# marcomistretta/incremental_multimodal_medical_learning_II

Hardware: AMD Instinct MI355X
Metric: contrastive train-step images/sec at global batch 1024; 1/2/4/8-GPU scaling (higher is better)
Workload: dtype bf16x3

## Files before the change

### incremental_multimodal_medical_learning_ii_amd/csrc/conv_wgrad.hip

```cpp
#include "conv_common.h"

using namespace cxrk;

namespace {
__global__ __launch_bounds__(256) void wgrad_reduce_bn_kernel(const float* __restrict__ slabs, int nslab, long slab_stride,
                                                              int taps, int C, int Cpad, const float* __restrict__ w,
                                                              const float* __restrict__ scale, float* __restrict__ dw,
                                                              float* __restrict__ dotpart, int accumulate, int sg_log2) {
  __shared__ float sh[16];
  __shared__ float4 red[256];
  const int ko = blockIdx.x;
  const int n = taps * Cpad;
  const float sc = scale ? scale[ko] : 1.f;
  const int SG = 1 << sg_log2, QPB = 256 >> sg_log2;
  const int ql = threadIdx.x & (QPB - 1), grp = threadIdx.x >> (8 - sg_log2);
  const int i4 = (blockIdx.y * QPB + ql) * 4;
  float4 s = make_float4(0.f, 0.f, 0.f, 0.f);
  if (i4 < n) {
    const float* src = slabs + (long)ko * n + i4;
    int z = grp;
    for (; z + 3 * SG < nslab; z += 4 * SG) {
      const float4 t0 = *reinterpret_cast<const float4*>(src + (long)z * slab_stride);
      const float4 t1 = *reinterpret_cast<const float4*>(src + (long)(z + SG) * slab_stride);
      const float4 t2 = *reinterpret_cast<const float4*>(src + (long)(z + 2 * SG) * slab_stride);
      const float4 t3 = *reinterpret_cast<const float4*>(src + (long)(z + 3 * SG) * slab_stride);
      s.x += (t0.x + t1.x) + (t2.x + t3.x); s.y += (t0.y + t1.y) + (t2.y + t3.y);
      s.z += (t0.z + t1.z) + (t2.z + t3.z); s.w += (t0.w + t1.w) + (t2.w + t3.w);
    }
    for (; z < nslab; z += SG) {
      const float4 t = *reinterpret_cast<const float4*>(src + (long)z * slab_stride);
      s.x += t.x; s.y += t.y; s.z += t.z; s.w += t.w;
    }
  }
  if (SG > 1) {
    red[threadIdx.x] = s;
    __syncthreads();
    if (grp == 0) {
      for (int g2 = 1; g2 < SG; ++g2) { const float4 t = red[g2 * QPB + ql]; s.x += t.x; s.y += t.y; s.z += t.z; s.w += t.w; }
    }
  }
  float dot = 0.f;
  if (i4 < n && grp == 0) {
    const int tap = i4 / Cpad, c = i4 - tap * Cpad;
    const float sv[4] = {s.x, s.y, s.z, s.w};
#pragma unroll
    for (int q = 0; q < 4; ++q) {
      if (c + q < C) {
        const long o = ((long)ko * taps + tap) * C + c + q;
        if (dotpart) dot += w[o] * sv[q];
        dw[o] = accumulate ? dw[o] + sc * sv[q] : sc * sv[q];
      }
    }
  }
  if (dotpart) {
    dot = block_sum(dot, sh);
    if (threadIdx.x == 0) dotpart[(long)ko * gridDim.y + blockIdx.y] = dot;
  }
}
__global__ void bn_param_grad_kernel(const float* __restrict__ dotpart, int nparts, const float* __restrict__ rstd,
                                     const float* __restrict__ rmean, const float* __restrict__ sumdy, int Ko,
                                     float* __restrict__ dgamma, float* __restrict__ dbeta, int accumulate) {
  const int ko = blockIdx.x * blockDim.x + threadIdx.x;
  if (ko >= Ko) return;
  float dot = 0.f;
  for (int p = 0; p < nparts; ++p) dot += dotpart[(long)ko * nparts + p];
  const float g = rstd[ko] * (dot - rmean[ko] * sumdy[ko]);
  dgamma[ko] = accumulate ? dgamma[ko] + g : g;
  dbeta[ko] = accumulate ? dbeta[ko] + sumdy[ko] : sumdy[ko];
}

}

static int wgrad_splitk(int Ko, int Ncols, long Kred, bool planes) { return wgrad_splitk_policy(Ko, Ncols, (int)Kred, planes); }
static int wgrad_dot_parts(int Nc) { return ceil_div(Nc, 64); }

extern "C" size_t cxrk_conv_wgrad_ws_bytes(int N, int H, int W, int C, int Ko, int R, int S, int stride, int pad) {
  const ConvGeom g = make_geom(N, H, W, C, Ko, R, S, stride, pad);
  int sk = wgrad_splitk(Ko, R * S * C, (long)N * g.Ho * g.Wo, false);
  const int sk2 = wgrad_splitk(Ko, R * S * C, (long)N * g.Ho * g.Wo, true);
  if (sk2 > sk) sk = sk2;
  return ((size_t)sk * (size_t)Ko * (size_t)(R * S * C) + (size_t)Ko * wgrad_dot_parts(R * S * C)) * sizeof(float);
}

template <class FMT>
static int conv_bwd_params_impl(const typename FMT::T* x, long xplane, const typename FMT::T* dy, long dyplane, const float* w,
                                const float* scale, const float* rstd, const float* rmean, const float* sumdy, float* dw,
                                float* dgamma, float* dbeta, int accumulate, int N, int H, int W, int C, int Cpad, int Ko, int R,
                                int S, int stride, int pad, float* ws, size_t ws_bytes, hipStream_t stream) {
  CXRK_CHECK_ARG(x && dy && dw && N > 0 && Cpad % FMT::EPL == 0 && Ko % FMT::EPL == 0 && aligned16(x) && aligned16(dy));
  CXRK_CHECK_ARG(!(dgamma && !(w && rstd && rmean && sumdy && dbeta)));
  const ConvGeom g = make_geom(N, H, W, Cpad, Ko, R, S, stride, pad);
  const long Kl = (long)N * g.Ho * g.Wo;
  CXRK_CHECK_ARG(Kl < (1L << 31));
  const int Kred = (int)Kl, Nc = R * S * Cpad;
  if ((long)H * W * Cpad * 4 * 3 >= (1L << 31)) return CXRK_ERR_UNSUPPORTED;
  int sk = wgrad_splitk(Ko, Nc, Kl, FMT::PLANES);
  const size_t slab_floats = (size_t)sk * Ko * Nc;
  CXRK_CHECK_WS(ws, ws_bytes, (slab_floats + (size_t)Ko * wgrad_dot_parts(Nc)) * sizeof(float));
  EpiParams ep{};
  ep.C = ws; ep.ldc = Nc; ep.alpha = 1.f; ep.slab_stride = (long)Ko * Nc;
  int rc;
  const bool exact = false;
  if (use_wide256(Ko, Nc, Kred, sk, FMT::PLANES)) {
    if constexpr (FMT::PLANES) {
      DmaDenseMC<256, 8>::P pa{dy, (long)Ko, Ko, Kred, dyplane}; DmaConvIm2colMC<256, 8>::P pb{x, g, Nc, Kred, xplane};
      rc = launch_gemm_pw<Pw256, DmaDenseMC<256, 8>, DmaConvIm2colMC<256, 8>>(pa, pb, ep, Ko, Nc, Kred, sk, stream);
    } else return CXRK_ERR_UNSUPPORTED;
  } else if (Ko <= 64) {
    if constexpr (FMT::PLANES) {
      DmaDenseMC<64, 4>::P pa{dy, (long)Ko, Ko, Kred, dyplane}; DmaConvIm2colMC<256, 4>::P pb{x, g, Nc, Kred, xplane};
      rc = launch_gemm_pw<Pw64x256, DmaDenseMC<64, 4>, DmaConvIm2colMC<256, 4>>(pa, pb, ep, Ko, Nc, Kred, sk, stream);
    } else {
      typename DenseMC<64, FMT>::P pa{dy, (long)Ko, Ko, Kred, dyplane}; typename ConvIm2colMC<256, FMT>::P pb{x, g, Nc, Kred, xplane};
      rc = launch_gemm<DenseMC<64, FMT>, ConvIm2colMC<256, FMT>, 1, 4>(pa, pb, ep, Ko, Nc, Kred, sk, stream, exact);
    }
  } else if constexpr (FMT::PLANES) {
    DmaDenseMC<128, 4>::P pa{dy, (long)Ko, Ko, Kred, dyplane}; DmaConvIm2colMC<128, 4>::P pb{x, g, Nc, Kred, xplane};
    rc = launch_gemm_pw<Pw128, DmaDenseMC<128, 4>, DmaConvIm2colMC<128, 4>>(pa, pb, ep, Ko, Nc, Kred, sk, stream);
  } else {
    typename DenseMC<128, FMT>::P pa{dy, (long)Ko, Ko, Kred, dyplane}; typename ConvIm2colMC<128, FMT>::P pb{x, g, Nc, Kred, xplane};
    rc = launch_gemm<DenseMC<128, FMT>, ConvIm2colMC<128, FMT>, 2, 2>(pa, pb, ep, Ko, Nc, Kred, sk, stream, exact);
  }
  if (rc < 0) return rc;
  const int sg_log2 = rc >= 64 ? 4 : (rc >= 8 ? 2 : 0);
  const int ny = ceil_div(Nc, 4 * (256 >> sg_log2));
  float* dotpart = dgamma ? ws + slab_floats : nullptr;
  hipLaunchKernelGGL(wgrad_reduce_bn_kernel, dim3(Ko, ny), dim3(256), 0, stream, ws, rc, (long)Ko * Nc, R * S, C, Cpad, w, scale, dw,
                     dotpart, accumulate, sg_log2);
  CXRK_LAUNCH_CHECK();
  if (dgamma) {
    hipLaunchKernelGGL(bn_param_grad_kernel, dim3(ceil_div(Ko, 256)), dim3(256), 0, stream, dotpart, ny, rstd, rmean, sumdy, Ko, dgamma,
                       dbeta, accumulate);
    CXRK_LAUNCH_CHECK();
  }
  return CXRK_OK;
}

extern "C" int cxrk_conv_bn_act_bwd_params(const float* x, const float* dy, const float* w, const float* scale,
                                           const float* rstd, const float* rmean, const float* sumdy, float* dw,
                                           float* dgamma, float* dbeta, int accumulate, int N, int H, int W, int C,
                                           int Cpad, int Ko, int R, int S, int stride, int pad, float* ws, size_t ws_bytes,
                                           hipStream_t stream) {
  return conv_bwd_params_impl<F32>(x, 0, dy, 0, w, scale, rstd, rmean, sumdy, dw, dgamma, dbeta, accumulate, N, H, W, C, Cpad, Ko, R, S,
                                   stride, pad, ws, ws_bytes, stream);
}
extern "C" int cxrk_conv_bn_act_bwd_params_pl(const void* x, long xplane, const void* dy, long dyplane, const float* w,
                                              const float* scale, const float* rstd, const float* rmean, const float* sumdy,
                                              float* dw, float* dgamma, float* dbeta, int accumulate, int N, int H, int W, int C,
                                              int Ko, int R, int S, int stride, int pad, float* ws, size_t ws_bytes,
                                              hipStream_t stream) {
  return conv_bwd_params_impl<PL>(static_cast<const unsigned short*>(x), xplane, static_cast<const unsigned short*>(dy), dyplane, w, scale,
                                  rstd, rmean, sumdy, dw, dgamma, dbeta, accumulate, N, H, W, C, C, Ko, R, S, stride, pad, ws, ws_bytes,
                                  stream);
}
```

### incremental_multimodal_medical_learning_ii_amd/kernels.py

```python
from __future__ import annotations

from typing import NamedTuple, Optional, Tuple

import torch

from . import _lib
from ._lib import check

ACT_NONE, ACT_RELU, ACT_GELU = 0, 1, 2
AUX_NONE, AUX_RELU_MASK, AUX_GELU_GRAD, AUX_MASK_BITS = 0, 1, 2, 3


def _stream() -> int:
    return torch.cuda.current_stream().cuda_stream


def _p(t: Optional[torch.Tensor]) -> Optional[int]:
    return None if t is None else t.data_ptr()


def _chk(t: torch.Tensor, name: str, dtype=torch.float32) -> torch.Tensor:
    if not isinstance(t, torch.Tensor) or not t.is_cuda:
        raise ValueError(f"{name}: expected a tensor on the GPU (the cxrk path has no CPU fallback), got "
                         f"{type(t).__name__} on {getattr(t, 'device', None)}")
    if t.dtype != dtype:
        raise ValueError(f"{name}: expected dtype {dtype}, got {t.dtype}")
    return t


def _chk_out(t, shape, name: str, dtype=torch.float32):
    if isinstance(t, Planes):
        if tuple(t.shape) != tuple(shape) or not t.is_contiguous():
            raise ValueError(f"{name}: expected contiguous Planes of shape {tuple(shape)}, got {tuple(t.shape)}")
        return t
    _chk(t, name, dtype)
    if tuple(t.shape) != tuple(shape) or not t.is_contiguous():
        raise ValueError(f"{name}: expected a contiguous tensor of shape {tuple(shape)}, got {tuple(t.shape)} strides {t.stride()}")
    return t


def _rowmajor2d(t: torch.Tensor, name: str) -> Tuple[torch.Tensor, int]:
    _chk(t, name)
    if t.dim() != 2:
        raise ValueError(f"{name}: expected 2-D, got shape {tuple(t.shape)}")
    if t.shape[1] != 1 and t.stride(1) != 1:
        t = t.contiguous()
    return t, (t.stride(0) if t.shape[0] > 1 else max(t.shape[1], t.stride(0)))


class Planes:
    __slots__ = ("t",)

    def __init__(self, t: torch.Tensor):
        if t.dtype != torch.bfloat16 or t.dim() < 2 or t.shape[0] != 2 or not t.is_cuda:
            raise ValueError(f"Planes: expected a bf16 GPU tensor [2, ...], got {t.dtype} {tuple(t.shape)} on {t.device}")
        self.t = t

    @staticmethod
    def empty(*shape, device) -> "Planes":
        return Planes(torch.empty((2,) + tuple(shape), dtype=torch.bfloat16, device=device))

    @staticmethod
    def zeros(*shape, device) -> "Planes":
        return Planes(torch.zeros((2,) + tuple(shape), dtype=torch.bfloat16, device=device))

    @property
    def shape(self):
        return self.t.shape[1:]

    @property
    def device(self):
        return self.t.device

    @property
    def plane(self) -> int:
        return self.t.stride(0)

    def ptr(self) -> int:
        return self.t.data_ptr()

    def numel(self) -> int:
        return self.t.numel() // 2

    def view(self, *shape) -> "Planes":
        return Planes(self.t.view((2,) + tuple(shape)))

    def rows(self, sl) -> "Planes":
        return Planes(self.t[:, sl])

    def is_contiguous(self) -> bool:
        return self.t[0].is_contiguous()

    def float(self) -> torch.Tensor:
        if self.is_contiguous() and self.numel() % 8 == 0:
            out = torch.empty(tuple(self.shape), dtype=torch.float32, device=self.t.device)
            check(_lib.load().cxrk_merge_planes(self.ptr(), self.plane, self.numel(), _p(out), _stream()), "cxrk_merge_planes")
            return out
        return self.t[0].float() + self.t[1].float()


def split_planes(x: torch.Tensor, out: Optional[Planes] = None) -> Planes:
    _chk(x, "split_planes.x")
    x = x.contiguous()
    if out is None:
        out = Planes.empty(*x.shape, device=x.device)
    check(_lib.load().cxrk_split_planes(_p(x), x.numel(), out.ptr(), out.plane, _stream()), "cxrk_split_planes")
    return out


def _pl2d(t: Planes, name: str):
    if not isinstance(t, Planes) or len(t.shape) != 2:
        raise ValueError(f"{name}: expected a 2-D Planes tensor")
    v = t.t
    if v.shape[2] != 1 and v.stride(2) != 1:
        raise ValueError(f"{name}: planes columns must be contiguous")
    return v.data_ptr(), (v.stride(1) if v.shape[1] > 1 else max(v.shape[2], v.stride(1))), v.stride(0)


class LaunchProfiler:

    PEAK_BF16X3, PEAK_F32, PEAK_HBM = 2500e12 / 3.0, 157.3e12, 8.0e12

    def __init__(self):
        self.on = False
        self.rows = []

    def start(self):
        self.on, self.rows = True, []

    def stop(self):
        self.on = False

    def bracket(self, key: str, flops: float, nbytes: float = 0.0, sub: int = 1):
        if not self.on:
            return None
        a, b = torch.cuda.Event(enable_timing=True), torch.cuda.Event(enable_timing=True)
        a.record()
        self.rows.append((key, flops, nbytes, a, b, sub))
        return b

    def summary(self):
        out = {}
        for key, flops, nbytes, a, b, sub in self.rows:
            d = out.setdefault(key, {"launches": 0, "flops": 0.0, "bytes": 0.0, "ms": 0.0, "floor_ms": 0.0})
            d["launches"] += sub
            d["flops"] += flops
            d["bytes"] += nbytes
            d["ms"] += a.elapsed_time(b)
            peak = self.PEAK_BF16X3 if (key.startswith("gemm_pw") or key.startswith("gemm_x3")) else self.PEAK_F32
            d["floor_ms"] += 1e3 * max(flops / peak, nbytes / self.PEAK_HBM)
        return out


profiler = LaunchProfiler()
# ... 359 lines not shown
    op, opl = _fmt(dz, "bn_train_dz.dz")
    check(lib.cxrk_bn_train_dz(dp, dpl, zp, zpl, _p(_vec(A, C, "A")), _p(_vec(B, C, "B")), _p(_vec(Cc, C, "Cc")), op, opl, rows, C, _stream()),
          "cxrk_bn_train_dz")
    return dz



def bn_fold(w, gamma, beta, rmean, rvar, eps, Ko, taps, C, Cpad, w_scaled, scale, shift, rstd):
    lib = _lib.load()
    for n, t in (("w", w), ("gamma", gamma), ("beta", beta), ("rmean", rmean), ("rvar", rvar)):
        _chk(t, "bn_fold." + n)
    check(lib.cxrk_bn_fold(_p(w), _p(gamma), _p(beta), _p(rmean), _p(rvar), float(eps), Ko, taps, C, Cpad,
                           _p(w_scaled), _p(scale), _p(shift), _p(rstd), _stream()), "cxrk_bn_fold")


def conv_fwd(x, w_scaled, shift, residual, y, N, H, W, C, Ko, R, S, stride, pad, relu):
    lib = _lib.load()
    ev = None
    if profiler.on:
        Ho, Wo = (H + 2 * pad - R) // stride + 1, (W + 2 * pad - S) // stride + 1
        fl = 2.0 * N * Ho * Wo * Ko * R * S * C
        ev = profiler.bracket(_label("ConvIm2colKC", "DenseKC", "4,1" if Ko <= 64 else "2,2", N * Ho * Wo, Ko, R * S * C, 1,
                                     1 if C % 32 == 0 else 3), fl,
                              4.0 * (N * H * W * C + Ko * R * S * C + N * Ho * Wo * Ko * (1 + (residual is not None))))
    rc = lib.cxrk_conv_bn_act_fwd(_p(_chk(x, "conv.x")), _p(w_scaled), _p(shift), _p(residual), _p(y), N, H, W, C, Ko,
                                  R, S, stride, pad, int(relu), _stream())
    if ev is not None:
        ev.record()
    check(rc, f"cxrk_conv_bn_act_fwd(N={N},H={H},W={W},C={C},Ko={Ko},R={R},s={stride})")
    return y


def _conv_out(H, W, R, S, stride, pad):
    return (H + 2 * pad - R) // stride + 1, (W + 2 * pad - S) // stride + 1


def _dgrad_label(N, H, W, Ko, R, S, stride):
    if stride == 1:
        return "ConvDgradKC", "ConvFilterMC", N * H * W, R * S * Ko, 1
    classes = 4 if R > 1 else 1
    return "ConvDgradS2KC", "ConvFilterS2MC", N * ((H + 1) // 2) * ((W + 1) // 2), Ko * max(1, (R * S) // 4), classes


def conv_bwd_data(dy, w_scaled, residual, relu_src, dx, N, H, W, C, Ko, R, S, stride, pad, sums=None):
    lib = _lib.load()
    ws = workspace(lib.cxrk_conv_bwd_data_colsum_ws_bytes(N, H, W, C, stride), dy.device) if sums is not None else None
    ev = None
    if profiler.on:
        Ho, Wo = _conv_out(H, W, R, S, stride, pad)
        fl = 2.0 * N * Ho * Wo * Ko * R * S * C
        la, lb, Ml, Kl, sub = _dgrad_label(N, H, W, Ko, R, S, stride)
        ev = profiler.bracket(_label(la, lb, "4,1" if C <= 64 else "2,2", Ml, C, Kl, 1, 2), fl,
                              4.0 * (N * Ho * Wo * Ko + Ko * R * S * C + N * H * W * C * (1 + (residual is not None) + (relu_src is not None))), sub)
    rc = lib.cxrk_conv_bn_act_bwd_data(_p(_chk(dy, "conv.dy")), _p(w_scaled), _p(residual), _p(relu_src), _p(dx), N, H,
                                       W, C, Ko, R, S, stride, pad, _p(sums), _p(ws), ws.numel() * 4 if ws is not None else 0, _stream())
    if ev is not None:
        ev.record()
    check(rc, f"cxrk_conv_bn_act_bwd_data(N={N},H={H},W={W},C={C},Ko={Ko},R={R},s={stride})")
    return dx


def conv_bwd_params(x, dy, w, scale, rstd, rmean, sumdy, dw, dgamma, dbeta, accumulate, N, H, W, C, Cpad, Ko, R, S, stride, pad):
    lib = _lib.load()
    wsb = lib.cxrk_conv_wgrad_ws_bytes(N, H, W, Cpad, Ko, R, S, stride, pad)
    ws = workspace(wsb, x.device)
    ev = None
    if profiler.on:
        Ho, Wo = _conv_out(H, W, R, S, stride, pad)
        fl = 2.0 * N * Ho * Wo * Ko * R * S * Cpad
        sk = lib.cxrk_gemm_wgrad_splitk(Ko, R * S * Cpad, N * Ho * Wo, 0)
        ev = profiler.bracket(_label("DenseMC", "ConvIm2colMC", "1,4" if Ko <= 64 else "2,2", Ko, R * S * Cpad, N * Ho * Wo, sk, 0,
                                     False), fl, 4.0 * (N * H * W * Cpad + N * Ho * Wo * Ko + Ko * R * S * Cpad))
    check(lib.cxrk_conv_bn_act_bwd_params(_p(_chk(x, "conv.x")), _p(_chk(dy, "conv.dy")), _p(w), _p(scale), _p(rstd),
                                          _p(rmean), _p(sumdy), _p(dw), _p(dgamma), _p(dbeta), int(accumulate), N, H, W,
                                          C, Cpad, Ko, R, S, stride, pad, _p(ws), ws.numel() * 4, _stream()),
          f"cxrk_conv_bn_act_bwd_params(N={N},H={H},W={W},C={C},Ko={Ko},R={R},s={stride})")
    if ev is not None:
        ev.record()



def bn_fold_pl(w, gamma, beta, rmean, rvar, eps, Ko, taps, C, Cpad, w_scaled: Planes, scale, shift, rstd):
    lib = _lib.load()
    for n, t in (("w", w), ("gamma", gamma), ("beta", beta), ("rmean", rmean), ("rvar", rvar)):
        _chk(t, "bn_fold." + n)
    check(lib.cxrk_bn_fold_pl(_p(w), _p(gamma), _p(beta), _p(rmean), _p(rvar), float(eps), Ko, taps, C, Cpad, w_scaled.ptr(),
                              w_scaled.plane, _p(scale), _p(shift), _p(rstd), _stream()), "cxrk_bn_fold_pl")


def conv_fwd_pl(x, w_scaled, shift, residual: Optional[Planes], y: Planes, maskout, N, H, W, C, Ko, R, S, stride, pad, relu):
    lib = _lib.load()
    in_planes = isinstance(x, Planes)
    if in_planes != isinstance(w_scaled, Planes):
        raise ValueError("conv_fwd_pl: x and w_scaled must share the storage format")
    ev = None
    if profiler.on:
        Ho, Wo = _conv_out(H, W, R, S, stride, pad)
        fl = 2.0 * N * Ho * Wo * Ko * R * S * C
        nb = 4.0 * (N * H * W * C + Ko * R * S * C + N * Ho * Wo * Ko * (1 + (residual is not None))) + (N * Ho * Wo * Ko / 8.0 if maskout is not None else 0.0)
        if in_planes:
            key = _label("ConvIm2colKC", "DenseKC", "4,1" if Ko <= 64 else "2,2", N * Ho * Wo, Ko, R * S * C, 1, 1, planes=True)
        else:
            key = _label("ConvIm2colKC", "DenseKC", "4,1" if Ko <= 64 else "2,2", N * Ho * Wo, Ko, R * S * C, 1, 3)
        ev = profiler.bracket(key, fl, nb)
    if maskout is not None:
        _chk(maskout, "conv.maskout", torch.uint8)
    xp, xpl = (x.ptr(), x.plane) if in_planes else (_p(_chk(x, "conv.x")), 0)
    wp, wpl = (w_scaled.ptr(), w_scaled.plane) if in_planes else (_p(_chk(w_scaled, "conv.w")), 0)
    rc = lib.cxrk_conv_bn_act_fwd_pl(xp, xpl, wp, wpl, int(in_planes), _p(shift), residual.ptr() if residual is not None else None,
                                     residual.plane if residual is not None else 0, y.ptr(), y.plane, _p(maskout), N, H, W, C, Ko, R, S,
                                     stride, pad, int(relu), _stream())
    if ev is not None:
        ev.record()
    check(rc, f"cxrk_conv_bn_act_fwd_pl(N={N},H={H},W={W},C={C},Ko={Ko},R={R},s={stride})")
    return y


def conv_bwd_data_pl(dy: Planes, w_scaled: Planes, residual: Optional[Planes], maskin, dx: Planes, N, H, W, C, Ko, R, S, stride, pad,
                     sums=None, residual_s2: bool = False):
    lib = _lib.load()
    if residual_s2:
        if residual is None or tuple(residual.shape) != (N, (H + 1) // 2, (W + 1) // 2, C):
            raise ValueError(f"conv_bwd_data_pl: compact residual must be [N, (H+1)//2, (W+1)//2, C], got {None if residual is None else tuple(residual.shape)}")
    ws = workspace(lib.cxrk_conv_bwd_data_colsum_ws_bytes(N, H, W, C, stride), dy.device) if sums is not None else None
    ev = None
    if profiler.on:
        Ho, Wo = _conv_out(H, W, R, S, stride, pad)
        fl = 2.0 * N * Ho * Wo * Ko * R * S * C
        la, lb, Ml, Kl, sub = _dgrad_label(N, H, W, Ko, R, S, stride)
        ev = profiler.bracket(_label(la, lb, "4,1" if C <= 64 else "2,2", Ml, C, Kl, 1, 2, planes=True), fl,
                              4.0 * (N * Ho * Wo * Ko + Ko * R * S * C + N * H * W * C * (1 + (0.0 if residual is None else 0.25 if residual_s2 else 1.0)))
                              + (N * H * W * C / 8.0 if maskin is not None else 0.0), sub)
    fn = lib.cxrk_conv_bn_act_bwd_data_pl_s2res if residual_s2 else lib.cxrk_conv_bn_act_bwd_data_pl
    rc = fn(dy.ptr(), dy.plane, w_scaled.ptr(), w_scaled.plane, residual.ptr() if residual is not None else None,
                                          residual.plane if residual is not None else 0, _p(maskin), dx.ptr(), dx.plane, N, H, W, C, Ko, R, S,
                                          stride, pad, _p(sums), _p(ws), ws.numel() * 4 if ws is not None else 0, _stream())
    if ev is not None:
        ev.record()
    check(rc, f"cxrk_conv_bn_act_bwd_data_pl{'_s2res' if residual_s2 else ''}(N={N},H={H},W={W},C={C},Ko={Ko},R={R},s={stride})")
    return dx


def conv1x1_s2_bwd_data_compact_pl(dy: Planes, w_scaled: Planes, N, H, W, C, Ko) -> Optional[Planes]:
    Ho, Wo = (H + 1) // 2, (W + 1) // 2
    if N * Ho * Wo * C * 2 >= (1 << 31):
        return None
    if tuple(dy.shape) not in ((N, Ho, Wo, Ko), (N * Ho * Wo, Ko)) or tuple(w_scaled.shape) != (Ko, C):
        raise ValueError(f"conv1x1_s2_bwd_data_compact_pl: dy {tuple(dy.shape)}, w {tuple(w_scaled.shape)} for N={N},H={H},W={W},C={C},Ko={Ko}")
    out = Planes.empty(N * Ho * Wo, C, device=dy.device)
    linear_bwd_data_pl(dy.view(N * Ho * Wo, Ko), w_scaled, out=out)
    return out.view(N, Ho, Wo, C)


def conv_bwd_params_pl(x: Planes, dy: Planes, w, scale, rstd, rmean, sumdy, dw, dgamma, dbeta, accumulate, N, H, W, C, Ko, R, S, stride, pad):
    lib = _lib.load()
    ws = workspace(lib.cxrk_conv_wgrad_ws_bytes(N, H, W, C, Ko, R, S, stride, pad), x.device)
    ev = None
    if profiler.on:
        Ho, Wo = _conv_out(H, W, R, S, stride, pad)
        fl = 2.0 * N * Ho * Wo * Ko * R * S * C
        sk = lib.cxrk_gemm_wgrad_splitk(Ko, R * S * C, N * Ho * Wo, 1)
        ev = profiler.bracket(_label("DenseMC", "ConvIm2colMC", "1,4" if Ko <= 64 else "2,2", Ko, R * S * C, N * Ho * Wo, sk, 0, planes=True),
                              fl, 4.0 * (N * H * W * C + N * Ho * Wo * Ko + Ko * R * S * C))
    check(lib.cxrk_conv_bn_act_bwd_params_pl(x.ptr(), x.plane, dy.ptr(), dy.plane, _p(w), _p(scale), _p(rstd), _p(rmean), _p(sumdy),
                                             _p(dw), _p(dgamma), _p(dbeta), int(accumulate), N, H, W, C, Ko, R, S, stride, pad, _p(ws),
                                             ws.numel() * 4, _stream()),
          f"cxrk_conv_bn_act_bwd_params_pl(N={N},H={H},W={W},C={C},Ko={Ko},R={R},s={stride})")
    if ev is not None:
        ev.record()


def maxpool_fwd_pl(x: Planes):
    lib = _lib.load()
    N, H, W, C = x.shape
    Ho, Wo = (H - 1) // 2 + 1, (W - 1) // 2 + 1
    y = Planes.empty(N, Ho, Wo, C, device=x.device)
    idx = torch.empty(N, Ho, Wo, C, dtype=torch.uint8, device=x.device)
    check(lib.cxrk_maxpool_fwd_pl(x.ptr(), x.plane, y.ptr(), y.plane, _p(idx), N, H, W, C, _stream()), "cxrk_maxpool_fwd_pl")
    return y, idx


def maxpool_bwd_pl(dy: Planes, idx, pooled: Planes, H: int, W: int) -> torch.Tensor:
    lib = _lib.load()
    N, _, _, C = pooled.shape
    dx = torch.empty(N, H, W, C, dtype=torch.float32, device=dy.device)
    check(lib.cxrk_maxpool_bwd_pl(dy.ptr(), dy.plane, _p(idx), pooled.ptr(), _p(dx), N, H, W, C, _stream()), "cxrk_maxpool_bwd_pl")
    return dx


def spatial_mean_bwd_pl(dy: torch.Tensor, Pn: int, add: Optional[torch.Tensor] = None) -> Planes:
    lib = _lib.load()
    N, C = dy.shape
    dx = Planes.empty(N, Pn, C, device=dy.device)
    if add is not None:
        add = _chk(add, "spatial_mean.add").contiguous()
    check(lib.cxrk_spatial_mean_bwd_pl(_p(_chk(dy.contiguous(), "spatial_mean.dy")), _p(add), dx.ptr(), dx.plane, N, Pn, C, _stream()),
          "cxrk_spatial_mean_bwd_pl")
    return dx


def unpack_mask(mask: torch.Tensor, C: int) -> torch.Tensor:
    m = mask.cpu().reshape(-1, C // 8).to(torch.int32)
    bits = (m.unsqueeze(-1) >> torch.arange(8, dtype=torch.int32)) & 1
    return bits.reshape(-1, C).bool()


def nchw_to_nhwc(x: torch.Tensor, cpad: int) -> torch.Tensor:
    lib = _lib.load()
    _chk(x, "nchw_to_nhwc.x")
    x = x.contiguous()
    N, C, H, W = x.shape
    y = torch.empty(N, H, W, cpad, dtype=torch.float32, device=x.device)
    check(lib.cxrk_nchw_to_nhwc(_p(x), _p(y), N, C, H, W, cpad, _stream()), "cxrk_nchw_to_nhwc")
    return y


def nhwc_to_nchw(x: torch.Tensor) -> torch.Tensor:
    lib = _lib.load()
    _chk(x, "nhwc_to_nchw.x")
    N, H, W, C = x.shape
    y = torch.empty(N, C, H, W, dtype=torch.float32, device=x.device)
    check(lib.cxrk_nhwc_to_nchw(_p(x), _p(y), N, C, H, W, _stream()), "cxrk_nhwc_to_nchw")
    return y


def _chk_images(x: torch.Tensor, name: str) -> torch.Tensor:
    _chk(x, name)
    if x.dim() != 4 or x.shape[1] not in (1, 3):
        raise ValueError(f"{name}: expected [N, 3, H, W] or [N, 1, H, W] images, got shape {tuple(x.shape)}")
    if x.requires_grad:
        raise ValueError(f"{name}: the augmentation has no input gradient; pass images that do not require grad")
    return x.contiguous()


def augment_params(x: torch.Tensor, spec, seed: int, counter: int, row_offset: int = 0, out: Optional[torch.Tensor] = None) -> torch.Tensor:
    lib = _lib.load()
    x = _chk_images(x, "augment_params.x")
    N, C, Hs, Ws = x.shape
    Ho, Wo = spec.size_for(Hs, Ws)
    params = torch.empty(N, 8, dtype=torch.float32, device=x.device) if out is None else _chk_out(out, (N, 8), "augment_params.out")
    check(lib.cxrk_augment_params(_p(x) if spec.contrast != 0 else None, N, C, Hs, Ws, Ho, Wo, spec.rotate_deg, spec.translate, spec.zoom[0],
                                  spec.zoom[1], spec.flip_p, spec.brightness, spec.contrast, int(seed) & (2 ** 64 - 1),
                                  int(counter) & 0xFFFFFFFF, int(row_offset), _p(params), _stream()), "cxrk_augment_params")
    return params


def augment_nhwc(x: torch.Tensor, cpad: int, params: torch.Tensor, out_size=None, clamp01: bool = False,
                 out: Optional[torch.Tensor] = None) -> torch.Tensor:
    lib = _lib.load()
    x = _chk_images(x, "augment_nhwc.x")
    N, C, Hs, Ws = x.shape
    Ho, Wo = (Hs, Ws) if out_size is None else (int(out_size[0]), int(out_size[1]))
    _chk(params, "augment_nhwc.params")
    if tuple(params.shape) != (N, 8) or not params.is_contiguous():
        raise ValueError(f"augment_nhwc.params: expected a contiguous [{N}, 8] tensor, got {tuple(params.shape)}")
    y = torch.empty(N, Ho, Wo, cpad, dtype=torch.float32, device=x.device) if out is None else _chk_out(out, (N, Ho, Wo, cpad), "augment_nhwc.out")
    check(lib.cxrk_augment_nhwc(_p(x), _p(params), _p(y), N, C, Hs, Ws, Ho, Wo, cpad, int(bool(clamp01)), _stream()), "cxrk_augment_nhwc")
    return y


def maxpool_fwd(x: torch.Tensor):
    lib = _lib.load()
    N, H, W, C = x.shape
    Ho, Wo = (H - 1) // 2 + 1, (W - 1) // 2 + 1
    y = torch.empty(N, Ho, Wo, C, dtype=torch.float32, device=x.device)
    idx = torch.empty(N, Ho, Wo, C, dtype=torch.uint8, device=x.device)
    check(lib.cxrk_maxpool_fwd(_p(_chk(x, "maxpool.x")), _p(y), _p(idx), N, H, W, C, _stream()), "cxrk_maxpool_fwd")
    return y, idx


def maxpool_bwd(dy, idx, x, relu_mask: bool):
    lib = _lib.load()
    N, H, W, C = x.shape
    dx = torch.empty_like(x)
    check(lib.cxrk_maxpool_bwd(_p(_chk(dy, "maxpool.dy")), _p(idx), _p(x), _p(dx), N, H, W, C, int(relu_mask), _stream()),
          "cxrk_maxpool_bwd")
    return dx


def spatial_mean_fwd(x: torch.Tensor) -> torch.Tensor:
    lib = _lib.load()
    N, Pn, C = x.shape
    y = torch.empty(N, C, dtype=torch.float32, device=x.device)
    check(lib.cxrk_spatial_mean_fwd(_p(_chk(x, "spatial_mean.x")), _p(y), N, Pn, C, _stream()), "cxrk_spatial_mean_fwd")
    return y


def spatial_mean_bwd(dy: torch.Tensor, Pn: int) -> torch.Tensor:
    lib = _lib.load()
    N, C = dy.shape
    dx = torch.empty(N, Pn, C, dtype=torch.float32, device=dy.device)
    check(lib.cxrk_spatial_mean_bwd(_p(_chk(dy.contiguous(), "spatial_mean.dy")), _p(dx), N, Pn, C, _stream()),
          "cxrk_spatial_mean_bwd")
    return dx



def _new_out(rows, cols, device, planes: bool):
    if planes:
        o = Planes.empty(rows, cols, device=device)
        return o, o.ptr(), o.plane
    o = torch.empty(rows, cols, dtype=torch.float32, device=device)
    return o, o.data_ptr(), 0


class Drop(NamedTuple):
    seed: int
    counter: int
    layer: int
    site: int
    row_offset: int
    p: float

    def args(self):
        return (self.seed & (2 ** 64 - 1), self.counter & 0xFFFFFFFF, self.layer, self.site, self.row_offset, float(self.p))

# ... 486 lines not shown
```

Baseline: 6750.

## Add halo-window 3x3 weight-gradient kernel that reuses input rows instead of im2col

Adds a specialized 3x3 stride-1 weight-gradient kernel for 64-channel layers. Producer waves stream a ring buffer of input pixel rows plus dy tiles into LDS, and consumer waves build all nine tap fragments from shifted ring addresses, using a per-pixel boundary mask in place of im2col gathers. When split-K exceeds the CU count, the extra slabs go to a row-split variant. It is meant to cut redundant input loads and im2col address work for early ResNet stages, at the cost of a large hand-pipelined kernel with tricky synchronisation and boundary handling.

```diff
diff --git a/incremental_multimodal_medical_learning_ii_amd/csrc/conv_halo_wgrad.h b/incremental_multimodal_medical_learning_ii_amd/csrc/conv_halo_wgrad.h
--- /dev/null
+++ b/incremental_multimodal_medical_learning_ii_amd/csrc/conv_halo_wgrad.h
@@ -0,0 +1,225 @@
+#pragma once
+#include "conv_halo.h"
+
+namespace cxrk {
+
+constexpr int WG_RING = 256;
+constexpr int WG_XPLANE = (WG_RING + 8) * 128;
+constexpr int WG_ZERO = WG_RING * 128;
+constexpr int WG_NSD = 4;
+constexpr int WG_DPLANE = 32 * 128;
+constexpr int WG_DSTAGE = 2 * WG_DPLANE;
+constexpr int WG_NCW = 12, WG_NLW = 4;
+constexpr int WG_NT = 64 * (WG_NCW + WG_NLW);
+constexpr int WG_LDS = 2 * WG_XPLANE + WG_NSD * WG_DSTAGE + WG_NSD * 32 * 4;
+static_assert(HALO_MAXW + 1 < 64, "a K-tile's halo must stay within two 32-pixel groups on either side");
+
+template <bool ROW>
+__global__ __launch_bounds__(WG_NT) void conv3x3_wgrad_window_kernel(const unsigned short* __restrict__ x, long xplane,
+                                                                    const unsigned short* __restrict__ dy, long dyplane,
+                                                                    float* __restrict__ slabs, long slab_stride, int ldc, int M, int H, int W,
+                                                                    int nKt, int tiles_per_slab, int slab0) {
+  __shared__ __attribute__((aligned(1024))) unsigned char smem[WG_LDS];
+  const int tid = threadIdx.x;
+  const int lane = tid & 63;
+  const int wave = __builtin_amdgcn_readfirstlane(tid >> 6);
+  unsigned char* sX = smem;
+  unsigned char* sD = smem + 2 * WG_XPLANE;
+  unsigned* sMask = reinterpret_cast<unsigned*>(smem + 2 * WG_XPLANE + WG_NSD * WG_DSTAGE);
+  const int slab = slab0 + (ROW ? (int)blockIdx.x / 3 : (int)blockIdx.x);
+  const int kt0 = slab * tiles_per_slab, kt1 = min(nKt, kt0 + tiles_per_slab);
+  const int nT = kt1 - kt0;
+  const int P0 = kt0 * 32;
+  const int Pend = min(M, kt1 * 32);
+  const int W1 = W + 1;
+#define WG_BARRIER() do { __builtin_amdgcn_s_barrier(); asm volatile("" ::: "memory"); } while (0)
+
+  if (wave >= WG_NCW) {
+    const int L = (wave - WG_NCW) & 1, G = (wave - WG_NCW) >> 1;
+    int kk[2]; unsigned voff[2];
+#pragma unroll
+    for (int j = 0; j < 2; ++j) {
+      kk[j] = (2 * G + j) * 8 + (lane >> 3);
+      const int lc = (lane & 7) ^ (((kk[j] >> 1) & 1) << 2);
+      voff[j] = (unsigned)(kk[j] * 128 + lc * 16);
+    }
+    const int xlo = max(0, P0 - W1), xhi = min(M, Pend + W1);
+    auto issue_x = [&](int g) {
+      const long p0 = (long)P0 + 32 * g;
+      const __amdgpu_buffer_rsrc_t rs = tile_rsrc(x + L * xplane + p0 * HALO_CH);
+      unsigned char* dst = sX + L * WG_XPLANE + (g & 7) * 4096 + 2 * G * 1024;
+#pragma unroll
+      for (int j = 0; j < 2; ++j) {
+        const long p = p0 + kk[j];
+        dma16(rs, dst + j * 1024, (p >= xlo && p < xhi) ? voff[j] : VOFF_OOB);
+      }
+    };
+    auto issue_d = [&](int t) {
+      const long p0 = (long)P0 + 32 * t;
+      const __amdgpu_buffer_rsrc_t rs = tile_rsrc(dy + L * dyplane + p0 * 64);
+      unsigned char* dst = sD + (t & (WG_NSD - 1)) * WG_DSTAGE + L * WG_DPLANE + 2 * G * 1024;
+#pragma unroll
+      for (int j = 0; j < 2; ++j) dma16(rs, dst + j * 1024, (p0 + kk[j] < Pend) ? voff[j] : VOFF_OOB);
+    };
+    const bool masker = wave == WG_NCW;
+    int mw = 0, mh = 0, mm = P0 + (lane & 31);
+    if (masker) { mw = mm % W; mh = (mm / W) % H; }
+    const int stepr = 32 % W, stepq = (32 / W) % H;
+    auto write_mask = [&](int t) {
+      unsigned hv = 0, wv = 0;
+#pragma unroll
+      for (int d = 0; d < 3; ++d) {
+        if ((unsigned)(mh + d - 1) < (unsigned)H) hv |= 7u << (3 * d);
+        if ((unsigned)(mw + d - 1) < (unsigned)W) wv |= 0x49u << d;
+      }
+      sMask[(t & (WG_NSD - 1)) * 32 + (lane & 31)] = mm < M ? (hv & wv) : 0u;
+      mm += 32; mw += stepr; mh += stepq;
+      if (mw >= W) { mw -= W; ++mh; }
+      if (mh >= H) mh -= H;
+    };
+    for (int g = -2; g <= 4; ++g) issue_x(g);
+    for (int t = 0; t < WG_NSD - 1; ++t) issue_d(t);
+    if (masker) for (int t = 0; t < WG_NSD - 1; ++t) write_mask(t);
+    asm volatile("s_waitcnt vmcnt(0) lgkmcnt(0)" ::: "memory");
+    WG_BARRIER();
+#pragma unroll 1
+    for (int t = 0; t < nT; ++t) {
+      asm volatile("s_waitcnt vmcnt(8) lgkmcnt(0)" ::: "memory");
+      WG_BARRIER();
+      issue_x(t + 5);
+      issue_d(t + 3);
+      if (masker) write_mask(t + 3);
+    }
+    asm volatile("s_waitcnt vmcnt(0)" ::: "memory");
+    return;
+  }
+
+  if (tid < 64) *reinterpret_cast<unsigned*>(smem + (tid >> 5) * WG_XPLANE + WG_ZERO + (tid & 31) * 4) = 0u;
+  constexpr int NTAP = ROW ? 1 : 3;
+  const int kh = wave & 1, ch = (wave >> 1) & 1;
+  const int r = ROW ? (int)blockIdx.x % 3 : wave >> 2;
+  const int s0 = ROW ? wave >> 2 : 0;
+  const int g = lane >> 4, q = (lane & 15) >> 2, pp = lane & 3;
+  const int colx = ch * 64 + 32 * (g & 1) + 8 * pp;
+  const int dead = WG_ZERO + colx;
+  int prow[4], live[4][NTAP], ad[4][NTAP];
+#pragma unroll
+  for (int u = 0; u < 4; ++u) {
+    prow[u] = 16 * (u >> 1) + 8 * (g >> 1) + q + 4 * (u & 1);
+#pragma unroll
+    for (int s = 0; s < NTAP; ++s) {
+      const int rr = prow[u] + (r - 1) * W + s0 + s - 1;
+      live[u][s] = ((rr & (WG_RING - 1)) << 7) | (colx ^ ((rr & 2) << 5));
+    }
+  }
+  auto select = [&](const unsigned (&mk)[4]) {
+#pragma unroll
+    for (int u = 0; u < 4; ++u)
+#pragma unroll
+      for (int s = 0; s < NTAP; ++s) {
+        const int sel = (int)(mk[u] << (31 - (3 * r + s0 + s))) >> 31;
+        ad[u][s] = dead ^ ((live[u][s] ^ dead) & sel);
+        live[u][s] = (live[u][s] + 32 * 128) & (WG_RING * 128 - 1);
+      }
+  };
+  f32x16 acc[NTAP];
+#pragma unroll
+  for (int s = 0; s < NTAP; ++s)
+#pragma unroll
+    for (int e = 0; e < 16; ++e) acc[s][e] = 0.f;
+
+  typedef s16x4 __attribute__((address_space(3))) * lds_v4;
+  auto tr2 = [&](const unsigned char* a0, const unsigned char* a1) {
+    const s16x4 x0 = __builtin_amdgcn_ds_read_tr16_b64_v4i16((lds_v4)(a0));
+    const s16x4 x1 = __builtin_amdgcn_ds_read_tr16_b64_v4i16((lds_v4)(a1));
+    const s16x8 v = {x0[0], x0[1], x0[2], x0[3], x1[0], x1[1], x1[2], x1[3]};
+    return __builtin_bit_cast(bf16x8, v);
+  };
+  struct BFrag { bf16x8 h[2], l[2]; };
+  auto read_b = [&](BFrag& f, int s) {
+#pragma unroll
+    for (int kc = 0; kc < 2; ++kc) {
+      f.h[kc] = tr2(sX + ad[2 * kc][s], sX + ad[2 * kc + 1][s]);
+      f.l[kc] = tr2(sX + WG_XPLANE + ad[2 * kc][s], sX + WG_XPLANE + ad[2 * kc + 1][s]);
+    }
+  };
+  bf16x8 ah[2], al[2];
+  auto mfma6 = [&](f32x16& c, const BFrag& f) {
+#pragma unroll
+    for (int kc = 0; kc < 2; ++kc) {
+      c = __builtin_amdgcn_mfma_f32_32x32x16_bf16(al[kc], f.h[kc], c, 0, 0, 0);
+      c = __builtin_amdgcn_mfma_f32_32x32x16_bf16(ah[kc], f.l[kc], c, 0, 0, 0);
+      c = __builtin_amdgcn_mfma_f32_32x32x16_bf16(ah[kc], f.h[kc], c, 0, 0, 0);
+    }
+  };
+  auto read_mask = [&](unsigned (&mk)[4], int t) {
+#pragma unroll
+    for (int u = 0; u < 4; ++u) mk[u] = sMask[(t & (WG_NSD - 1)) * 32 + prow[u]];
+  };
+
+  asm volatile("s_waitcnt lgkmcnt(0)" ::: "memory");
+  WG_BARRIER();
+  {
+    unsigned mk[4];
+    read_mask(mk, 0);
+    select(mk);
+  }
+#pragma unroll 1
+  for (int t = 0; t < nT; ++t) {
+    asm volatile("s_waitcnt lgkmcnt(0)" ::: "memory");
+    WG_BARRIER();
+    const unsigned char* dt = sD + (t & (WG_NSD - 1)) * WG_DSTAGE;
+    BFrag B0, B1;
+#pragma unroll
+    for (int kc = 0; kc < 2; ++kc) {
+      ah[kc] = pw_frag_mc<64>(dt, kh * 32, kc, lane);
+      al[kc] = pw_frag_mc<64>(dt + WG_DPLANE, kh * 32, kc, lane);
+    }
+    read_b(B0, 0);
+    if constexpr (!ROW) read_b(B1, 1);
+    unsigned mk[4];
+    read_mask(mk, t + 1);
+    mfma6(acc[0], B0);
+    if constexpr (!ROW) read_b(B0, 2);
+    select(mk);
+    if constexpr (!ROW) { mfma6(acc[1], B1); mfma6(acc[NTAP - 1], B0); }
+  }
+  float* out = slabs + (long)slab * slab_stride;
+#pragma unroll
+  for (int s = 0; s < NTAP; ++s) {
+    const int col = (r * 3 + s0 + s) * HALO_CH + ch * 32 + (lane & 31);
+#pragma unroll
+    for (int e = 0; e < 16; ++e) {
+      const int row = kh * 32 + (e & 3) + 8 * (e >> 2) + 4 * (lane >> 5);
+      out[(long)row * ldc + col] = acc[s][e];
+    }
+  }
+#undef WG_BARRIER
+}
+
+static inline bool halo_wgrad_enabled() { const char* e = getenv("CXRK_HALO_WGRAD"); return e ? atoi(e) != 0 : true; }
+static inline bool halo_wgrad_shape(int N, int H, int W, int C, int Ko, int R, int S, int stride, int pad) {
+  return R == 3 && S == 3 && stride == 1 && pad == 1 && C == HALO_CH && Ko == 64 && W >= 1 && W <= HALO_MAXW && H >= 1 && N >= 1 &&
+         (long)N * H * W < (1L << 31) - 4096;
+}
+static int launch_conv3x3_wgrad_window(const unsigned short* x, long xplane, const unsigned short* dy, long dyplane, float* slabs, long slab_stride,
+                                       int ldc, int M, int H, int W, int splitk, hipStream_t stream) {
+  if (M <= 0 || W > HALO_MAXW || W < 1 || H < 1) return CXRK_ERR_ARG;
+  int kchunk = M;
+  if (splitk > 1) { kchunk = ceil_div(ceil_div(M, splitk), BK) * BK; splitk = ceil_div(M, kchunk); }
+  else splitk = 1;
+  const int nKt = ceil_div(M, 32);
+  const int tiles = splitk > 1 ? kchunk / 32 : nKt;
+  const int nfull = splitk < halo_cus() ? splitk : halo_cus();
+  hipLaunchKernelGGL(conv3x3_wgrad_window_kernel<false>, dim3((unsigned)nfull), dim3(WG_NT), 0, stream, x, xplane, dy, dyplane, slabs, slab_stride,
+                     ldc, M, H, W, nKt, tiles, 0);
+  CXRK_LAUNCH_CHECK();
+  if (splitk > nfull) {
+    hipLaunchKernelGGL(conv3x3_wgrad_window_kernel<true>, dim3((unsigned)(3 * (splitk - nfull))), dim3(WG_NT), 0, stream, x, xplane, dy, dyplane,
+                       slabs, slab_stride, ldc, M, H, W, nKt, tiles, nfull);
+    CXRK_LAUNCH_CHECK();
+  }
+  return splitk;
+}
+
+}
diff --git a/incremental_multimodal_medical_learning_ii_amd/csrc/conv_wgrad.hip b/incremental_multimodal_medical_learning_ii_amd/csrc/conv_wgrad.hip
--- a/incremental_multimodal_medical_learning_ii_amd/csrc/conv_wgrad.hip
+++ b/incremental_multimodal_medical_learning_ii_amd/csrc/conv_wgrad.hip
@@ -1,4 +1,5 @@
 #include "conv_common.h"
+#include "conv_halo_wgrad.h"
 
 using namespace cxrk;
 
@@ -94,6 +95,8 @@
   CXRK_CHECK_ARG(Kl < (1L << 31));
   const int Kred = (int)Kl, Nc = R * S * Cpad;
   if ((long)H * W * Cpad * 4 * 3 >= (1L << 31)) return CXRK_ERR_UNSUPPORTED;
+  const bool window = FMT::PLANES && halo_wgrad_enabled() && halo_wgrad_shape(N, H, W, Cpad, Ko, R, S, stride, pad) &&
+                      halo_applies(H, W, Cpad, Ko, R, S, stride, pad);
   int sk = wgrad_splitk(Ko, Nc, Kl, FMT::PLANES);
   const size_t slab_floats = (size_t)sk * Ko * Nc;
   CXRK_CHECK_WS(ws, ws_bytes, (slab_floats + (size_t)Ko * wgrad_dot_parts(Nc)) * sizeof(float));
@@ -101,7 +104,10 @@
   ep.C = ws; ep.ldc = Nc; ep.alpha = 1.f; ep.slab_stride = (long)Ko * Nc;
   int rc;
   const bool exact = false;
-  if (use_wide256(Ko, Nc, Kred, sk, FMT::PLANES)) {
+  if (window) {
+    if constexpr (FMT::PLANES) rc = launch_conv3x3_wgrad_window(x, xplane, dy, dyplane, ws, ep.slab_stride, Nc, Kred, H, W, sk, stream);
+    else return CXRK_ERR_UNSUPPORTED;
+  } else if (use_wide256(Ko, Nc, Kred, sk, FMT::PLANES)) {
     if constexpr (FMT::PLANES) {
       DmaDenseMC<256, 8>::P pa{dy, (long)Ko, Ko, Kred, dyplane}; DmaConvIm2colMC<256, 8>::P pb{x, g, Nc, Kred, xplane};
       rc = launch_gemm_pw<Pw256, DmaDenseMC<256, 8>, DmaConvIm2colMC<256, 8>>(pa, pb, ep, Ko, Nc, Kred, sk, stream);
diff --git a/incremental_multimodal_medical_learning_ii_amd/kernels.py b/incremental_multimodal_medical_learning_ii_amd/kernels.py
--- a/incremental_multimodal_medical_learning_ii_amd/kernels.py
+++ b/incremental_multimodal_medical_learning_ii_amd/kernels.py
@@ -1,5 +1,6 @@
 from __future__ import annotations
 
+import os
 from typing import NamedTuple, Optional, Tuple
 
 import torch
@@ -665,6 +666,17 @@
     return out.view(N, Ho, Wo, C)
 
 
+def _wgrad_window_takes(H, W, C, Ko, R, S, stride, pad) -> bool:
+    def off(name):
+        v = os.environ.get(name)
+        try:
+            return v is not None and int(v) == 0
+        except ValueError:
+            return True
+    return (R == 3 and S == 3 and stride == 1 and pad == 1 and C == 64 and Ko == 64 and 1 <= W <= 58 and H >= 1
+            and not off("CXRK_HALO") and not off("CXRK_HALO_WGRAD"))
+
+
 def conv_bwd_params_pl(x: Planes, dy: Planes, w, scale, rstd, rmean, sumdy, dw, dgamma, dbeta, accumulate, N, H, W, C, Ko, R, S, stride, pad):
     lib = _lib.load()
     ws = workspace(lib.cxrk_conv_wgrad_ws_bytes(N, H, W, C, Ko, R, S, stride, pad), x.device)
@@ -673,8 +685,11 @@
         Ho, Wo = _conv_out(H, W, R, S, stride, pad)
         fl = 2.0 * N * Ho * Wo * Ko * R * S * C
         sk = lib.cxrk_gemm_wgrad_splitk(Ko, R * S * C, N * Ho * Wo, 1)
-        ev = profiler.bracket(_label("DenseMC", "ConvIm2colMC", "1,4" if Ko <= 64 else "2,2", Ko, R * S * C, N * Ho * Wo, sk, 0, planes=True),
-                              fl, 4.0 * (N * H * W * C + N * Ho * Wo * Ko + Ko * R * S * C))
+        if _wgrad_window_takes(H, W, C, Ko, R, S, stride, pad):
+            label = "conv3x3_wgrad_window_kernel"
+        else:
+            label = _label("DenseMC", "ConvIm2colMC", "1,4" if Ko <= 64 else "2,2", Ko, R * S * C, N * Ho * Wo, sk, 0, planes=True)
+        ev = profiler.bracket(label, fl, 4.0 * (N * H * W * C + N * Ho * Wo * Ko + Ko * R * S * C))
     check(lib.cxrk_conv_bn_act_bwd_params_pl(x.ptr(), x.plane, dy.ptr(), dy.plane, _p(w), _p(scale), _p(rstd), _p(rmean), _p(sumdy),
                                              _p(dw), _p(dgamma), _p(dbeta), int(accumulate), N, H, W, C, Ko, R, S, stride, pad, _p(ws),
                                              ws.numel() * 4, _stream()),
```

Result: faster. 6827 (median of 6 runs) (+1.2%).
